# MP-Gadget/shenqi

Hardware: AMD Instinct MI355X
Metric: particle-steps/sec (grav+PM+SPH) at 256^3; rms force error vs ref (higher is better)
Workload: dtype f64

## Files before the change

include/shenqi_hip.h:

```cpp
#ifndef SHENQI_HIP_H
#define SHENQI_HIP_H

#include <stddef.h>
#include <stdint.h>

#ifdef __cplusplus
extern "C" {
#endif

#define SHQ_OK 0
#define SHQ_ERR_INVALID 1
#define SHQ_ERR_DEVICE 2
#define SHQ_ERR_NOMEM 3
#define SHQ_ERR_STATE 4
#define SHQ_ERR_NOCONV 5

#define SHQ_NGRAVTAB 512
#define SHQ_NMAXCHILD 8
#define SHQ_NODELISTLENGTH 4
#define SHQ_TIMEBINS 46

typedef struct shq_context shq_context;


// ... 363 lines not shown
    void *base;
    size_t elsize;
    int64_t numslots;
    size_t off_mintimebin, off_timebindynfric, off_jumptominpot;
    size_t off_dfaccel, off_df_surroundingvel, off_dragaccel;
    size_t off_minpotpos, off_minpotvel;
} shq_bh_dyn_view;
int shq_bh_dynamics_upload(shq_context *ctx, const shq_part_view *parts, const shq_bh_dyn_view *bh);
int shq_bh_dynamics_download(shq_context *ctx, const shq_part_view *parts, const shq_bh_dyn_view *bh);
int shq_set_bh_reposition(shq_context *ctx, int enabled);
int shq_kick_bh(shq_context *ctx, const double gravkick[SHQ_TIMEBINS + 1], const int32_t *active, int64_t nactive);
int shq_grav_short_run(shq_context *ctx, const shq_grav_params *params, const int32_t *active,
                       int64_t nactive, int update_potential, int walk_mode);
int shq_grav_short_run_range(shq_context *ctx, const shq_grav_params *params, int64_t first, int64_t count,
                             int update_potential, int walk_mode);
int shq_set_walk_stats(shq_context *ctx, int level);
int shq_set_walk_launch(shq_context *ctx, int persist, int leaf_ring);
int shq_set_walk_sparse(shq_context *ctx, int enable);
int shq_walk_pair_lean(shq_context *ctx);
int shq_set_walk_overlap(shq_context *ctx, int mode);
int shq_set_walk_addr(shq_context *ctx, int mode);
int shq_walk_last_addr(shq_context *ctx, int *mode);
int shq_walk_addr32_fits(int64_t numnodes);
int shq_walk_pair_status(shq_context *ctx, int64_t *recovered_launches, int64_t *stack_high_water, int64_t *last_mopped_tasks);
int shq_set_walk_debug(shq_context *ctx, int pair_spin_max, int pair_stack_cap);
int shq_set_tree_debug(shq_context *ctx, int64_t initial_node_cap);
int shq_tree_build_attempts(shq_context *ctx, int *attempts);
int shq_direct_force_sample(shq_context *ctx, const double *sample_pos, int64_t ns, int64_t nsrc, double BoxSize, double G, double h,
                            int repeat, double *accel);
int shq_grav_short_download(shq_context *ctx, double (*accel)[3], double *potential,
                            int64_t *ninteractions, shq_walk_stats *stats);
typedef struct shq_grav_query {
    double Pos[3];
    int32_t NodeList[4];
    double OldAcc;
} shq_grav_query;
typedef struct shq_grav_result {
    double Acc[3];
    double Potential;
} shq_grav_result;
int shq_grav_short_secondary(shq_context *ctx, const shq_grav_params *params, const shq_grav_query *queries, int64_t nq,
                             shq_grav_result *results, int64_t *ninteractions, int update_potential);
typedef struct shq_data_index {
    int32_t Task;
    int32_t Index;
    int32_t NodeList[4];
// ... 991 lines not shown
```

shenqi_amd/capi.py:

```python
import ctypes as C
import os

import numpy as np

_HERE = os.path.dirname(os.path.abspath(__file__))
LIBDIR = os.environ.get("SHQ_LIBDIR") or os.path.join(_HERE, "lib")
DATADIR = os.path.join(_HERE, "data")

NGRAVTAB = 512
NMAXCHILD = 8
NOFIELD = C.c_size_t(-1).value

WALK_EXACT = 0
WALK_GROUP = 1
WALK_AUTO = 2
WALK_TREE_ORDER = 0x100
WALK_DEFER_POSTPROCESS = 0x200


class ShqError(RuntimeError):
    """Non-zero status from the library (the shim's endrun() equivalent)."""


def _load(name):
# ... 394 lines not shown
GAS_NCOL = 28
hip.shq_gas_set_device.argtypes = [_vp, _vp, C.c_int64, C.c_int64]
hip.shq_gas_get_device.argtypes = [_vp, _vp, C.c_int64, C.c_int]
hip.shq_density_resident.argtypes = [_vp, C.POINTER(DensityParams), C.POINTER(SphStats)]
hip.shq_hydro_resident.argtypes = [_vp, C.POINTER(HydroParams), C.POINTER(SphStats)]
for _f in ("shq_gas_set_device", "shq_gas_get_device", "shq_density_resident", "shq_hydro_resident"):
    getattr(hip, _f).restype = C.c_int
hip.shq_set_walk_stats.argtypes = [_vp, C.c_int]
hip.shq_set_walk_stats.restype = C.c_int
hip.shq_set_walk_launch.argtypes = [_vp, C.c_int, C.c_int]
hip.shq_set_walk_launch.restype = C.c_int
hip.shq_set_walk_sparse.argtypes = [_vp, C.c_int]
hip.shq_set_walk_sparse.restype = C.c_int
hip.shq_walk_pair_lean.argtypes = [_vp]
hip.shq_walk_pair_lean.restype = C.c_int
hip.shq_set_walk_overlap.argtypes = [_vp, C.c_int]
hip.shq_set_walk_overlap.restype = C.c_int
hip.shq_set_walk_addr.argtypes = [_vp, C.c_int]
hip.shq_set_walk_addr.restype = C.c_int
hip.shq_walk_last_addr.argtypes = [_vp, C.POINTER(C.c_int)]
hip.shq_walk_last_addr.restype = C.c_int
hip.shq_walk_addr32_fits.argtypes = [C.c_int64]
hip.shq_walk_addr32_fits.restype = C.c_int
hip.shq_pm_set_fft_transposed.argtypes = [_vp, C.c_int]
hip.shq_pm_set_fft_transposed.restype = C.c_int
hip.shq_walk_pair_status.argtypes = [_vp, C.POINTER(C.c_int64), C.POINTER(C.c_int64), C.POINTER(C.c_int64)]
hip.shq_walk_pair_status.restype = C.c_int
hip.shq_set_walk_debug.argtypes = [_vp, C.c_int, C.c_int]
hip.shq_set_walk_debug.restype = C.c_int
hip.shq_set_tree_debug.argtypes = [_vp, C.c_int64]
hip.shq_set_tree_debug.restype = C.c_int
hip.shq_tree_build_attempts.argtypes = [_vp, C.POINTER(C.c_int)]
hip.shq_tree_build_attempts.restype = C.c_int
hip.shq_direct_force_sample.argtypes = [_vp, _vp, C.c_int64, C.c_int64, C.c_double, C.c_double, C.c_double, C.c_int, _vp]
hip.shq_direct_force_sample.restype = C.c_int
hip.shq_exchange_plan.argtypes = [_vp, C.POINTER(ExchangeLayout), _vp, C.c_int64, _vp, C.c_int, C.c_int, C.c_int64, C.POINTER(C.c_int64), C.POINTER(C.c_int64), _vp]
hip.shq_exchange_pack.argtypes = [_vp, C.POINTER(ExchangeLayout), _vp, _vp, C.c_int64, _vp, C.c_int, _vp, _vp]
hip.shq_exchange_unpack.argtypes = [_vp, C.POINTER(ExchangeLayout), _vp, C.c_int64, _vp, _vp, _vp, C.c_int]
hip.shq_slots_gc.argtypes = [_vp, C.POINTER(ExchangeLayout), _vp, C.POINTER(C.c_int64), C.c_int64, _vp, _vp, _vp]
hip.shq_slots_gc_sorted.argtypes = [_vp, C.POINTER(ExchangeLayout), _vp, C.POINTER(C.c_int64), C.c_int64, _vp, _vp, _vp]
hip.shq_slots_split_particles.argtypes = [_vp, C.POINTER(ExchangeLayout), C.POINTER(SpawnLayout), _vp, C.POINTER(C.c_int64), C.c_int64, _vp, _vp, C.c_int64, _vp]
hip.shq_slots_convert.argtypes = [_vp, C.POINTER(ExchangeLayout), _vp, C.c_int64, C.c_int64, _vp, _vp, _vp, _vp, C.c_int64, C.c_int]
hip.shq_make_particle_stars.argtypes = [_vp, C.POINTER(ExchangeLayout), C.POINTER(StarSpawnLayout), _vp, C.c_int64, C.c_int64, _vp, _vp, _vp, _vp, _vp, C.c_int64, C.c_double]
hip.shq_blackhole_make_seeds.argtypes = [_vp, C.POINTER(ExchangeLayout), C.POINTER(BhSeedLayout), _vp, C.c_int64, C.c_int64, _vp, _vp, _vp, _vp, _vp, C.c_int64,
                                         C.c_double, C.c_double]
hip.shq_bh_accretion.argtypes = [_vp, C.POINTER(TreeView), C.POINTER(PartView), C.POINTER(SphView), C.POINTER(BhSlotView), _vp, _vp, C.c_int64, C.POINTER(KickFactors),
# ... 926 lines not shown
```

shenqi_amd/csrc/capi.hip:

```cpp
#include "common.hpp"
#include <stdarg.h>
#include <string.h>
#include <stdlib.h>
#include <math.h>
#include <thread>
#include <atomic>
#include <algorithm>

static thread_local char g_err[1024] = "";

void shq_set_error(const char *fmt, ...)
{
    va_list ap;
    va_start(ap, fmt);
    vsnprintf(g_err, sizeof(g_err), fmt, ap);
    va_end(ap);
}

extern "C" const char *shq_last_error(void) { return g_err; }
extern "C" const char *shq_version(void) { return "shenqi_hip 0.1 (gfx950)"; }

namespace {

template <typename F> void parallel_for(int64_t n, F f)
// ... 286 lines not shown
    return SHQ_OK;
}

extern "C" int shq_set_walk_overlap(shq_context *ctx, int mode)
{
    SHQ_CHECK(ctx, SHQ_ERR_INVALID, "null context");
    SHQ_CHECK(mode >= 0 && mode <= 2, SHQ_ERR_INVALID, "walk overlap mode %d", mode);
    ctx->walk_overlap = mode;
    return SHQ_OK;
}

extern "C" int shq_set_walk_addr(shq_context *ctx, int mode)
{
    SHQ_CHECK(ctx, SHQ_ERR_INVALID, "null context");
    SHQ_CHECK(mode == 0 || mode == 1, SHQ_ERR_INVALID, "walk addr mode %d", mode);
    ctx->walk_addr = mode;
    return SHQ_OK;
}

extern "C" int shq_walk_last_addr(shq_context *ctx, int *mode)
{
    SHQ_CHECK(ctx && mode, SHQ_ERR_INVALID, "null argument");
    *mode = ctx->last_walk_addr32 ? 1 : 0;
    return SHQ_OK;
}

extern "C" int shq_walk_pair_lean(shq_context *ctx)
{
    SHQ_CHECK(ctx, SHQ_ERR_INVALID, "null context");
    if(!ctx->node_lean_checked || !ctx->node_lean_bad.ptr)
        return 0;
    SHQ_HIP(hipSetDevice(ctx->device));
    int bad = 1;
    SHQ_HIP(hipMemcpyAsync(&bad, ctx->node_lean_bad.ptr, sizeof(int), hipMemcpyDeviceToHost, ctx->stream));
    SHQ_HIP(hipStreamSynchronize(ctx->stream));
    return bad == 0 ? 1 : 0;
}

extern "C" int shq_set_walk_launch(shq_context *ctx, int persist, int leaf_ring)
{
    SHQ_CHECK(ctx && persist >= 0 && persist <= 2 && (leaf_ring == 0 || leaf_ring == 1), SHQ_ERR_INVALID, "walk launch: persist 0..2, leaf_ring 0 or 1");
    ctx->walk_persist = persist;
    ctx->walk_ring = leaf_ring;
    return SHQ_OK;
}

// ... 1182 lines not shown
```

shenqi_amd/csrc/common.hpp:

```cpp
#ifndef SHQ_COMMON_HPP
#define SHQ_COMMON_HPP

#include <hip/hip_runtime.h>
#include <hipfft/hipfft.h>
#include <stdint.h>
#include <stdio.h>
#include <string>
#include <vector>
#include "../../include/shenqi_hip.h"
#include "yields_math.hpp"
#include "cooling_math.hpp"

void shq_set_error(const char *fmt, ...);
void shq_heiii_run_free(shq_context *ctx);

#define SHQ_HIP(call)                                                                          \
    do {                                                                                       \
        hipError_t e_ = (call);                                                                \
        if(e_ != hipSuccess) {                                                                 \
            shq_set_error("%s:%d: %s failed: %s", __FILE__, __LINE__, #call, hipGetErrorString(e_)); \
            return (e_ == hipErrorOutOfMemory) ? SHQ_ERR_NOMEM : SHQ_ERR_DEVICE;               \
        }                                                                                      \
    } while(0)

// ... 406 lines not shown
    DevBuf<double> slab_fac;
    bool ps_slab = false;
    bool have_types = false;

    shq_walk_stats last_stats = {};
    int walk_variant = 3;
    int walk_stats = 0;
    int walk_persist = 1;
    int walk_ring = 1;
    int num_cus = 256;
    DevBuf<unsigned int> walk_tasks;
    DevBuf<int4> sp_items, sp_stack;
    DevBuf<int32_t> sp_count;
    DevBuf<int> sp_flags;
    PinBuf<int> sp_host;
    int sp_stack_cap = 0;
    unsigned sp_spin_max = 0;
    int walk_sparse = 1;
    DevBuf<int> node_lean_bad;
    bool node_lean_checked = false;
    int walk_overlap = 1;
    int walk_addr = 1;
    bool last_walk_addr32 = false;
    bool sp_check_pending = false;
    int xcd_k = 32;
    float last_walk_ms = 0;
    int last_walk_mode = 0;

    PinBuf<char> stage;

    bool uvbg_keep = false;
    int uvbg_n = 0;
    std::vector<float> uvbg_j21, uvbg_xhi;
    double uvbg_ms[4] = {0, 0, 0, 0};
    DevBuf<double> uvbg_tw, uvbg_tabs, uvbg_part;
    DevBuf<int> uvbg_flag;
    int uvbg_tw_n = 0, uvbg_tabs_n = 0, uvbg_tabs_nr = 0;
    shq_heiii_stats heiii_stats = {};
    struct HeiiiRun {
        int phase = 0;
        struct CallScope *sc = nullptr;
        int64_t n = 0;
        double box = 0, a3inv = 0, du = 0;
        int64_t m = 0, nrows = 0, n_flash = 0;
        int cur = 0;
        double4 *E[2] = {nullptr, nullptr}, *S = nullptr;
// ... 312 lines not shown
```

shenqi_amd/csrc/grav_walk.hip:

```cpp
#include "common.hpp"
#include "pm_readout.hpp"
#include <utility>
#include <stdlib.h>

namespace {

struct WalkArgs {
    const NodeG *nodeG;
    const double4 *posm;
    const double4 *posm_leaf;
    const double *oldacc;
    const int32_t *targets;
    const int32_t *qstart;
    double *acc;
    double *pot;
    int32_t *nint;
    GravStatsDev *stats;
    long long ntargets;
    int root;
    double Box, invBox, halfBox;
    double rcut, rcut2;
    double h, h2, h_inv, h3_inv;
    double inv_celldx;
    double errtol, bh2;
// ... 86 lines not shown
    }
    ax = fma(dx, fac, ax);
    ay = fma(dy, fac, ay);
    az = fma(dz, fac, az);
}

template <bool POT>
__device__ __forceinline__ void leaf_particle(const double4 *__restrict__ tab, const double4 q, double px, double py,
                                              double pz, const WalkArgs &a, double &ax, double &ay, double &az,
                                              double &pot, const unsigned long long wrapm)
{
    double ex = q.x - px, ey = q.y - py, ez = q.z - pz;
    if(wrapm != 0ull) {
        ex = wrapd(ex, a.Box, a.invBox);
        ey = wrapd(ey, a.Box, a.invBox);
        ez = wrapd(ez, a.Box, a.invBox);
    }
    const double rr2 = fma(ez, ez, fma(ey, ey, ex * ex));
    apply_accn<POT>(tab, ex, ey, ez, rr2, q.w, a, ax, ay, az, pot);
}

#if defined(__HIP_DEVICE_COMPILE__)
#define SHQ_CONSTANT_AS __attribute__((address_space(4)))
#else
#define SHQ_CONSTANT_AS
#endif
typedef const SHQ_CONSTANT_AS WalkArgs *WalkArgsK;
__device__ __forceinline__ WalkArgsK walk_cold_args()
{
    WalkArgsK kp = (WalkArgsK) __builtin_amdgcn_kernarg_segment_ptr();
    asm volatile("" : "+s"(kp));
    return kp;
}

template <typename T> __device__ __forceinline__ void agent_store(T *p, T v) { __hip_atomic_store(p, v, __ATOMIC_RELAXED, __HIP_MEMORY_SCOPE_AGENT); }
template <typename T> __device__ __forceinline__ T agent_load(const T *p) { return __hip_atomic_load(const_cast<T *>(p), __ATOMIC_RELAXED, __HIP_MEMORY_SCOPE_AGENT); }

__device__ __forceinline__ int walk_next_task(WalkArgsK c, int &region, int &tried)
{
    const int lg = c->task_run_log2;
    const int nwaves = (int) c->nwaves;
    unsigned int *counters = c->task_counters;
    while(tried < 8) {
        unsigned k = 0;
        if((threadIdx.x & 63) == 0)
            k = atomicAdd(&counters[16 * region], 1u);
        k = (unsigned) __builtin_amdgcn_readfirstlane((int) k);
        const unsigned t = ((((k >> lg) << 3) + (unsigned) region) << lg) | (k & ((1u << lg) - 1u));
        if(k < 0x40000000u && t < (unsigned) nwaves)
            return (int) t;
        region = (region + 1) & 7;
        tried++;
    }
    return -1;
}

#define SHQ_LEAF_RING 32
#ifndef SHQ_SPARSE_LANES
#define SHQ_SPARSE_LANES 8
#endif
#ifndef SHQ_SPARSE_CAP
#define SHQ_SPARSE_CAP 96
#endif
#define SHQ_SPARSE_STACK 4096
#define SHQ_SPARSE_SPIN (1u << 22)
#ifndef SHQ_PAIR_DEPTH2
#define SHQ_PAIR_DEPTH2 1
#endif
enum SpFlag {
    SP_OVERFLOW = 0,
    SP_GAVEUP = 1,
    SP_MOPPED = 2,
    SP_HIGHWATER = 3,
    SP_STICKY_ERROR = 8,
    SP_STICKY_RECOVERED = 9,
    SP_STICKY_HIGHWATER = 10,
    SP_TASK_COUNTER = 16
};
#define SP_TASK_DONE (-2)
#ifndef SHQ_PAIR_WAVES
#define SHQ_PAIR_WAVES 8
#define SHQ_PAIR_WG_PER_CU 2
// ... 384 lines not shown
            atomicAdd(&c.stats->lonely[3], (unsigned long long) l16m);
        }
    }
    }
    wave = PERSIST ? (long long) walk_next_task(walk_cold_args(), region, tried) : -1;
    }
}

struct LeanProducts { double rcuthl, mlen2, inside, wraplim; };
__device__ __forceinline__ LeanProducts lean_products(double mass, double len, double rcut, double Box)
{
    LeanProducts r;
    const double hl = 0.5 * len;
    r.rcuthl = rcut + hl;
    r.mlen2 = mass * len * len;
    r.inside = 0.6 * len;
    r.wraplim = fmax(0.5 * Box - hl, 0.0);
    return r;
}
__device__ __forceinline__ int lean_level(double rootlen, double len) { return (__double2hiint(rootlen) - __double2hiint(len)) >> 20; }

#pragma clang diagnostic push
#pragma clang diagnostic ignored "-Wpass-failed"
template <bool POT, int WAVES>
__device__ __forceinline__ void grav_pair_body(const WalkArgs &a)
{
    __shared__ double4 tab[SHQ_NGRAVTAB];
    __shared__ double4 tgt_all[WAVES][64];
    __shared__ double acc_all[WAVES][4][64];
    __shared__ int cnt_all[WAVES][64];
    __shared__ double bh_lvl[32];
    if(a.sp_mop && agent_load(a.sp_flags + SP_GAVEUP) == 0)
        return;
    const double rootlen = a.Box * 1.001;
    if(threadIdx.x < 32) {
        const double l = ldexp(rootlen, -(int) threadIdx.x);
        bh_lvl[threadIdx.x] = l * l / a.bh2;
    }
    const bool lean = __builtin_amdgcn_readfirstlane(a.sp_lean_bad ? (*a.sp_lean_bad == 0) : 0) != 0;
    for(int i = threadIdx.x; i < SHQ_NGRAVTAB; i += blockDim.x) {
        const int j = (i + 1 < SHQ_NGRAVTAB) ? i + 1 : i;
        const double f0 = a.tab_f[i], f1 = a.tab_f[j], p0 = a.tab_p[i], p1 = a.tab_p[j];
        tab[i] = i + 1 < SHQ_NGRAVTAB ? make_double4(f0, f1 - f0, p0, p1 - p0) : make_double4(0, 0, 0, 0);
    }
    __syncthreads();
    const int lane = threadIdx.x & 63, wv = threadIdx.x >> 6;
    double4 *const tgt = tgt_all[wv];
    double(*const acc)[64] = acc_all[wv];
    int *const cntl = cnt_all[wv];
    int4 *const stack = a.sp_stack + ((size_t) blockIdx.x * WAVES + wv) * (size_t) a.sp_stack_cap;
    int sp_high = 0;
    int mopped = 0;
    const unsigned long long below = (1ull << lane) - 1ull;
    long long w_sum = 0, w_min = 0x7fffffffffffll, w_max = 0;
    auto next_task = [&](long long prev) -> long long {
        if(a.sp_live) {
            unsigned k = 0;
            if(lane == 0)
                k = atomicAdd(a.sp_task, 1u);
            return (long long) (unsigned) __builtin_amdgcn_readfirstlane((int) k);
        }
        return prev < 0 ? (long long) blockIdx.x * WAVES + wv : prev + (long long) gridDim.x * WAVES;
    };
    for(long long task = next_task(-1); task < a.nwaves; task = next_task(task)) {
        const long long t = task * 64 + lane;
        const bool valid = t < a.ntargets;
        const long long pi = valid ? (a.targets ? (long long) a.targets[t] : t) : -1;
        const bool have = pi >= 0;
        int cnt = agent_load(&a.sp_count[task]);
        if(a.sp_mop) {
            if(__builtin_amdgcn_readfirstlane(cnt) == SP_TASK_DONE)
                continue;
            mopped++;
        }
        if(a.sp_live) {
            for(unsigned spin = 0; cnt < 0 && spin < a.sp_spin_max; spin++) {
                __builtin_amdgcn_s_sleep(32);
                cnt = agent_load(&a.sp_count[task]);
            }
            cnt = __builtin_amdgcn_readfirstlane(cnt);
            if(cnt < 0) {
                if(lane == 0)
                    agent_store(a.sp_flags + SP_GAVEUP, 1);
                break;
            }
        }
        int sp = 0;
        if(cnt > 0) {
            double4 me = make_double4(0, 0, 0, 0);
            if(have) {
                const double4 p = a.posm[pi];
                me = make_double4(p.x, p.y, p.z, a.errtol * agent_load(&a.oldacc[pi]));
            }
            tgt[lane] = me;
            for(int k = 0; k < 4; k++)
                acc[k][lane] = 0.0;
            cntl[lane] = 0;
            for(int k0 = 0; k0 < cnt; k0 += 64) {
                int4 mine = make_int4(0, 0, 0, 0);
                if(k0 + lane < cnt) {
                    const unsigned long long *const it = reinterpret_cast<const unsigned long long *>(a.sp_items + (task * SHQ_SPARSE_CAP + k0 + lane));
                    const unsigned long long lo = agent_load(it), hi = agent_load(it + 1);
                    mine = make_int4((int) (unsigned) lo, (int) (unsigned) (lo >> 32), (int) (unsigned) hi, (int) (unsigned) (hi >> 32));
                }
                const int kn = cnt - k0 < 64 ? cnt - k0 : 64;
                for(int k = 0; k < kn; k++) {
                    const int ix = __builtin_amdgcn_readlane(mine.x, k), iy = __builtin_amdgcn_readlane(mine.y, k);
                    const unsigned long long m = ((unsigned long long) (unsigned) __builtin_amdgcn_readlane(mine.w, k) << 32) |
                                                 (unsigned) __builtin_amdgcn_readlane(mine.z, k);
                    if((m >> lane) & 1ull)
                        stack[sp + __popcll(m & below)] = make_int4(ix, iy, lane, 0);
                    sp += __popcll(m);
                }
            }
            __builtin_amdgcn_fence(__ATOMIC_RELEASE, "wavefront");
            __builtin_amdgcn_wave_barrier();
        }
        struct PairLd {
            int node, end, slot, kind;
            double4 src;
            double cx, cy, cz, len;
            int nsib, nchild, ntype, ncount;
        };
        struct PairOut {
            int push_sib, push_child, child_end, leaf0, leafn;
        };
        auto pair_pop = [&](int base, int np, PairLd &p) {
            p.node = -1, p.end = -1, p.slot = 0, p.kind = 0;
            if(lane < np) {
                const int4 pr = stack[base + lane];
                p.node = pr.x, p.end = pr.y, p.slot = pr.z, p.kind = pr.w;
            }
        };
        auto pair_fetch = [&](PairLd &p) {
            p.src = make_double4(0, 0, 0, 0);
            p.cx = p.cy = p.cz = p.len = 0;
            p.nsib = -1, p.nchild = -1, p.ntype = 0, p.ncount = 0;
            if(p.node >= 0) {
                const double4 *const sp4 = p.kind == 1 ? a.posm_leaf + p.node : reinterpret_cast<const double4 *>(a.nodeG + p.node);
                p.src = *sp4;
                if(p.kind == 0) {
                    const NodeG *const nd = a.nodeG + p.node;
                    p.len = nd->len;
                    p.cx = nd->center[0], p.cy = nd->center[1], p.cz = nd->center[2];
                    p.nsib = nd->sibling, p.nchild = nd->child, p.ntype = nd->type, p.ncount = nd->count;
                }
            }
        };
        auto pair_eval = [&](const PairLd &p, PairOut &o) {
            o.push_sib = -1, o.push_child = -1, o.child_end = -1, o.leaf0 = 0, o.leafn = 0;
            double ax = 0, ay = 0, az = 0, pot = 0;
            const bool live = p.node >= 0, isnode = live && p.kind == 0;
            double wraplim = 0, rcut2 = 0, rcuthl = 0, mlen2 = 0, bhlim = 0, inside = 0;
            if(isnode) {
                if(lean) {
                    const LeanProducts lp = lean_products(p.src.w, p.len, a.rcut, a.Box);
                    rcuthl = lp.rcuthl, mlen2 = lp.mlen2, inside = lp.inside, wraplim = lp.wraplim, rcut2 = a.rcut2;
                    bhlim = bh_lvl[lean_level(rootlen, p.len) & 31];
                } else {
                    const NodeG *const nd = a.nodeG + p.node;
                    bhlim = nd->bhlim, mlen2 = nd->mlen2, inside = nd->inside, rcut2 = nd->rcut2, wraplim = nd->wraplim, rcuthl = nd->rcuthl;
                }
            }
            const double4 tg = tgt[p.slot];
            double dx = p.src.x - tg.x, dy = p.src.y - tg.y, dz = p.src.z - tg.z;
            double ux = p.cx - tg.x, uy = p.cy - tg.y, uz = p.cz - tg.z;
            double cmax = fmax(fmax(fabs(ux), fabs(uy)), fabs(uz));
            const bool nwrap = isnode && __double2hiint(wraplim) >= 0 && cmax >= wraplim;
            if(nwrap || (live && !isnode)) {
                dx = wrapd(dx, a.Box, a.invBox);
                dy = wrapd(dy, a.Box, a.invBox);
                dz = wrapd(dz, a.Box, a.invBox);
            }
            if(nwrap) {
                ux = wrapd(ux, a.Box, a.invBox);
                uy = wrapd(uy, a.Box, a.invBox);
                uz = wrapd(uz, a.Box, a.invBox);
                cmax = fmax(fmax(fabs(ux), fabs(uy)), fabs(uz));
            }
            const double r2 = dx * dx + dy * dy + dz * dz;
            bool ev = live && !isnode;
            if(isnode) {
                const bool keep = !(r2 > rcut2 && cmax > rcuthl);
                const bool open = (!a.useBH && mlen2 > r2 * r2 * tg.w) || r2 < bhlim || cmax < inside;
                ev = keep && !open;
                if(keep && open) {
                    if(p.ntype == SHQ_NODE_NODE_TYPE) {
                        o.push_child = p.nchild;
                        o.child_end = p.nsib;
                    } else if(p.ntype == SHQ_PARTICLE_NODE_TYPE) {
                        o.leaf0 = p.nchild;
                        o.leafn = p.ncount;
                    }
                }
                if(p.nsib != p.end && p.nsib >= 0)
                    o.push_sib = p.nsib;
            }
            if(ev) {
                apply_accn<POT, true>(tab, dx, dy, dz, r2, p.src.w, a, ax, ay, az, pot);
                atomicAdd(&acc[0][p.slot], ax);
                atomicAdd(&acc[1][p.slot], ay);
                atomicAdd(&acc[2][p.slot], az);
                if(POT)
                    atomicAdd(&acc[3][p.slot], pot);
                atomicAdd(&cntl[p.slot], 1);
            }
        };
        auto push_nodes = [&](int what, int what_end, int slot) {
            const unsigned long long m = shq_ballot(what >= 0);
            if(what >= 0)
                stack[sp + __popcll(m & below)] = make_int4(what, what_end, slot, 0);
            sp += __popcll(m);
        };
        auto push_leaves = [&](int leaf0, int leafn, int slot) {
            if(shq_ballot(leafn > 0) != 0ull) {
                const unsigned long long b0 = shq_ballot((leafn & 1) != 0), b1 = shq_ballot((leafn & 2) != 0),
                                         b2 = shq_ballot((leafn & 4) != 0), b3 = shq_ballot((leafn & 8) != 0);
                const int off = __popcll(b0 & below) + 2 * __popcll(b1 & below) + 4 * __popcll(b2 & below) + 8 * __popcll(b3 & below);
                for(int k = 0; k < SHQ_NMAXCHILD; k++) {
                    if(shq_ballot(k < leafn) == 0ull)
                        break;
                    if(k < leafn)
                        stack[sp + off + k] = make_int4(leaf0 + k, -1, slot, 1);
                }
                sp += __popcll(b0) + 2 * __popcll(b1) + 4 * __popcll(b2) + 8 * __popcll(b3);
            }
        };
        while(sp > 0) {
            const int npa = sp < 64 ? sp : 64;
            sp -= npa;
            const int npb = SHQ_PAIR_DEPTH2 ? (sp < 64 ? sp : 64) : 0;
            sp -= npb;
            PairLd pa, pb;
            PairOut oa, ob;
            pair_pop(sp + npb, npa, pa);
            if(npb > 0)
                pair_pop(sp, npb, pb);
            pair_fetch(pa);
            if(npb > 0)
                pair_fetch(pb);
            pair_eval(pa, oa);
            if(npb > 0)
                pair_eval(pb, ob);
            push_nodes(oa.push_sib, pa.end, pa.slot);
            if(npb > 0)
                push_nodes(ob.push_sib, pb.end, pb.slot);
            push_nodes(oa.push_child, oa.child_end, pa.slot);
            if(npb > 0)
                push_nodes(ob.push_child, ob.child_end, pb.slot);
            push_leaves(oa.leaf0, oa.leafn, pa.slot);
            if(npb > 0)
                push_leaves(ob.leaf0, ob.leafn, pb.slot);
            sp_high = sp > sp_high ? sp : sp_high;
            if(sp > a.sp_stack_cap - 1280) {
                if(lane == 0) {
                    agent_store(a.sp_flags + SP_OVERFLOW, 1);
                    atomicOr(a.sp_flags + SP_STICKY_ERROR, 1);
                }
                sp = 0;
            }
            __builtin_amdgcn_fence(__ATOMIC_RELEASE, "wavefront");
            __builtin_amdgcn_wave_barrier();
        }
        long long nint = 0;
        if(have) {
            nint = agent_load(&a.nint[pi]);
            if(cnt > 0) {
                __builtin_amdgcn_fence(__ATOMIC_ACQUIRE, "wavefront");
                a.acc[3 * pi + 0] = agent_load(&a.acc[3 * pi + 0]) + acc[0][lane];
                a.acc[3 * pi + 1] = agent_load(&a.acc[3 * pi + 1]) + acc[1][lane];
                a.acc[3 * pi + 2] = agent_load(&a.acc[3 * pi + 2]) + acc[2][lane];
                if(POT)
                    a.pot[pi] = agent_load(&a.pot[pi]) + acc[3][lane];
                nint += (long long) cntl[lane];
                a.nint[pi] = (int32_t) nint;
            }
        }
        long long mn = have ? nint : 0x7fffffffffffll, mx = have ? nint : 0, sm = have ? nint : 0;
        for(int off = 32; off > 0; off >>= 1) {
            const long long o1 = __shfl_xor(mn, off), o2 = __shfl_xor(mx, off), o3 = __shfl_xor(sm, off);
            mn = o1 < mn ? o1 : mn;
            mx = o2 > mx ? o2 : mx;
            sm += o3;
        }
        w_sum += sm;
        w_min = mn < w_min ? mn : w_min;
        w_max = mx > w_max ? mx : w_max;
        if(lane == 0)
            agent_store(&a.sp_count[task], (int32_t) SP_TASK_DONE);
        __builtin_amdgcn_wave_barrier();
    }
    if(lane == 0 && a.stats) {
        atomicAdd(&a.stats->ninteractions, (unsigned long long) w_sum);
        atomicMin(&a.stats->min_int, w_min);
        atomicMax(&a.stats->max_int, w_max);
    }
    if(lane == 0 && sp_high > 0) {
        atomicMax(a.sp_flags + SP_HIGHWATER, sp_high);
        atomicMax(a.sp_flags + SP_STICKY_HIGHWATER, sp_high);
    }
    if(lane == 0 && mopped > 0)
        atomicAdd(a.sp_flags + SP_MOPPED, mopped);
    if(a.sp_mop && blockIdx.x == 0 && threadIdx.x == 0)
        atomicAdd(a.sp_flags + SP_STICKY_RECOVERED, 1);
}

template <bool POT> __global__ __launch_bounds__(256) __attribute__((amdgpu_waves_per_eu(4, 4))) void grav_pair_kernel_live(const WalkArgs a) { grav_pair_body<POT, 4>(a); }
template <bool POT> __global__ __launch_bounds__(64 * SHQ_PAIR_WAVES) __attribute__((amdgpu_waves_per_eu(SHQ_PAIR_EU, SHQ_PAIR_EU))) void grav_pair_kernel(const WalkArgs a)
{
    grav_pair_body<POT, SHQ_PAIR_WAVES>(a);
}

#pragma clang diagnostic pop

__global__ void grav_postprocess_kernel(const int32_t *targets, long long ntargets, const double4 *posm, double *acc,
                                        double *pot, double *treeacc, double G, double h, double cbrtrho0,
                                        int update_potential)
{
    const long long t = (long long) blockIdx.x * blockDim.x + threadIdx.x;
    if(t >= ntargets)
        return;
    const long long i = targets ? (long long) targets[t] : t;
    if(i < 0)
        return;
    const double a0 = acc[3 * i + 0] * G, a1 = acc[3 * i + 1] * G, a2 = acc[3 * i + 2] * G;
    acc[3 * i + 0] = a0;
    acc[3 * i + 1] = a1;
    acc[3 * i + 2] = a2;
    if(update_potential) {
        treeacc[3 * i + 0] = a0;
        treeacc[3 * i + 1] = a1;
        treeacc[3 * i + 2] = a2;
        const double m = posm[i].w;
// ... 78 lines not shown
        grav_walk_exact_kernel<POT, PREFETCH, LEAFB, (POT && !PREFETCH && LEAFB == 2) ? 2 : 1, BH><<<grid, block, 0, stream>>>(a);
    else if(stats)
        grav_walk_exact_kernel<POT, PREFETCH, LEAFB, 1, BH><<<grid, block, 0, stream>>>(a);
    else if(persist && !PREFETCH && LEAFB == 2 && block.x == 512)
        grav_walk_exact_kernel<POT, PREFETCH, LEAFB, 0, BH, false, (!PREFETCH && LEAFB == 2), (!PREFETCH && LEAFB == 2)><<<grid, block, dyn_lds, stream>>>(a);
    else if(persist && !PREFETCH && LEAFB == 2)
        grav_walk_exact_kernel<POT, PREFETCH, LEAFB, 0, BH, false, (!PREFETCH && LEAFB == 2)><<<grid, block, dyn_lds, stream>>>(a);
    else
        grav_walk_exact_kernel<POT, PREFETCH, LEAFB, 0, BH><<<grid, block, 0, stream>>>(a);
    return false;
}

template <bool POT, bool PREFETCH, int LEAFB>
bool launch_variant(int stats, bool persist, dim3 grid, dim3 block, hipStream_t stream, const WalkArgs &a, size_t dyn_lds = 0, bool addr32 = false)
{
    if(a.useBH)
        return launch_variant_bh<POT, PREFETCH, LEAFB, true>(stats, persist, grid, block, stream, a, dyn_lds, addr32);
    return launch_variant_bh<POT, PREFETCH, LEAFB, false>(stats, persist, grid, block, stream, a, dyn_lds, addr32);
}

}

extern "C" int shq_walk_addr32_fits(int64_t numnodes) { return (numnodes >= 0 && numnodes + 1 <= ((int64_t) 1 << 25)) ? 1 : 0; }

void shq_launch_stats_init(shq_context *ctx) { stats_init_kernel<<<1, 1, 0, ctx->stream>>>(ctx->gstats.ptr); }

void shq_fill_node_walk_params(shq_context *ctx, const shq_grav_params *p)
{
    if((ctx->node_rcut != p->Rcut || ctx->node_bh2 != p->BHOpeningAngle2) && ctx->numnodes > 0) {
        const long long n = ctx->numnodes + 1;
        int *lean_bad = nullptr;
        if(ctx->node_lean_bad.reserve(16) == SHQ_OK && hipMemsetAsync(ctx->node_lean_bad.ptr, 0, sizeof(int) * 16, ctx->stream) == hipSuccess)
            lean_bad = ctx->node_lean_bad.ptr;
        ctx->node_lean_checked = lean_bad != nullptr;
        fill_rcuthl_kernel<<<dim3((unsigned) ((n + 255) / 256)), dim3(256), 0, ctx->stream>>>(ctx->nodeG.ptr, n, p->Rcut, p->BHOpeningAngle2, p->BoxSize, lean_bad);
        ctx->node_rcut = p->Rcut;
        ctx->node_bh2 = p->BHOpeningAngle2;
    }
}

static void fill_walk_args(shq_context *ctx, const shq_grav_params *p, WalkArgs &a)
{
    shq_fill_node_walk_params(ctx, p);
    a.nodeG = ctx->nodeG.ptr;
    a.posm = ctx->posm.ptr;
    a.posm_leaf = ctx->posm_leaf.ptr;
// ... 312 lines not shown
    bool used32 = false;
    if(update_potential) {
        switch(variant) {
        case 0: launch_variant<true, false, 4>(stats, persist, grid, block, ctx->stream, a); break;
        case 1: launch_variant<true, false, 2>(stats, persist, grid, block, ctx->stream, a); break;
        case 2: launch_variant<true, false, 4>(stats, persist, grid, block, ctx->stream, a); break;
        default: used32 = launch_variant<true, false, 2>(stats, persist, grid, block, ctx->stream, a, dyn_lds, addr32); break;
        }
    } else {
        switch(variant) {
        case 0: launch_variant<false, false, 4>(stats, persist, grid, block, ctx->stream, a); break;
        case 1: launch_variant<false, false, 2>(stats, persist, grid, block, ctx->stream, a); break;
        case 2: launch_variant<false, false, 4>(stats, persist, grid, block, ctx->stream, a); break;
        default: used32 = launch_variant<false, false, 2>(stats, persist, grid, block, ctx->stream, a, dyn_lds, addr32); break;
        }
    }
    SHQ_HIP(hipGetLastError());
    ctx->last_walk_addr32 = used32;
    if(sparse) {
        hipStream_t ps = live ? ctx->stream_pair : ctx->stream;
        if(live)
            SHQ_HIP(hipStreamWaitEvent(ps, ctx->ev_pair_fork, 0));
        const dim3 pg((unsigned) pair_blocks);
        if(live) {
            if(update_potential)
                grav_pair_kernel_live<true><<<pg, dim3(256), 0, ps>>>(a);
            else
                grav_pair_kernel_live<false><<<pg, dim3(256), 0, ps>>>(a);
        } else if(update_potential)
            grav_pair_kernel<true><<<pg, dim3(64 * SHQ_PAIR_WAVES), 0, ps>>>(a);
        else
            grav_pair_kernel<false><<<pg, dim3(64 * SHQ_PAIR_WAVES), 0, ps>>>(a);
        SHQ_HIP(hipGetLastError());
        if(live) {
            SHQ_HIP(hipEventRecord(ctx->ev_pair_join, ps));
            SHQ_HIP(hipStreamWaitEvent(ctx->stream, ctx->ev_pair_join, 0));
            WalkArgs m = a;
            m.sp_live = 0;
            m.sp_mop = 1;
            const dim3 mg((unsigned) mop_blocks);
            if(update_potential)
                grav_pair_kernel<true><<<mg, dim3(64 * SHQ_PAIR_WAVES), 0, ctx->stream>>>(m);
            else
                grav_pair_kernel<false><<<mg, dim3(64 * SHQ_PAIR_WAVES), 0, ctx->stream>>>(m);
            SHQ_HIP(hipGetLastError());
        }
        SHQ_HIP(hipMemcpyAsync(ctx->sp_host.ptr, ctx->sp_flags.ptr + SP_STICKY_ERROR, sizeof(int) * 8, hipMemcpyDeviceToHost, ctx->stream));
        ctx->sp_check_pending = true;
    }
    SHQ_HIP(hipEventRecord(ctx->ev_end[SHQ_T_WALK], ctx->stream));
    if(swap_meshes) {
        std::swap(ctx->mesh.ptr, ctx->mesh_alt.ptr);
        std::swap(ctx->mesh.cap, ctx->mesh_alt.cap);
    }
    if(scrubbed)
        ctx->mesh_zeroed = true;
    return SHQ_OK;
}

int shq_launch_grav_postprocess(shq_context *ctx, const shq_grav_params *p, const int32_t *d_active, int64_t ntargets,
                                int update_potential, int64_t first)
{
    if(ntargets == 0)
        return SHQ_OK;
    const int threads = 256;
    const long long blocks = (ntargets + threads - 1) / threads;
    grav_postprocess_kernel<<<dim3((unsigned) blocks), dim3(threads), 0, ctx->stream>>>(
// ... 98 lines not shown
```

Baseline: 433.0 million.

## Use 32-bit offsets and wave-mask logic in sparse pair gravity walk

Adds an A32 variant of the pair-walk kernel that addresses the node table, leaf positions and per-wave stack with 32-bit byte offsets from uniform bases. Push and evaluation decisions become wave-wide ballot masks, with inverse_ballot masking and mbcnt-based prefix counts, and the leaf push is unrolled into mask-guarded stores. Per-task min/max/sum reductions move out of the task loop, and SHQ_SPARSE_LANES rises from 8 to 12. The aim is lower VGPR/SGPR pressure and less 64-bit address arithmetic and divergence, at the cost of more code and a size-fit check that falls back to 64-bit addressing.

```diff
diff --git a/include/shenqi_hip.h b/include/shenqi_hip.h
--- a/include/shenqi_hip.h
+++ b/include/shenqi_hip.h
@@ -409,6 +409,8 @@
 int shq_set_walk_addr(shq_context *ctx, int mode);
 int shq_walk_last_addr(shq_context *ctx, int *mode);
 int shq_walk_addr32_fits(int64_t numnodes);
+int shq_pair_addr32_fits(int64_t numnodes, int64_t leaf_slots, int64_t stack_cap);
+int shq_walk_last_pair_addr(shq_context *ctx, int *mode);
 int shq_walk_pair_status(shq_context *ctx, int64_t *recovered_launches, int64_t *stack_high_water, int64_t *last_mopped_tasks);
 int shq_set_walk_debug(shq_context *ctx, int pair_spin_max, int pair_stack_cap);
 int shq_set_tree_debug(shq_context *ctx, int64_t initial_node_cap);
diff --git a/shenqi_amd/capi.py b/shenqi_amd/capi.py
--- a/shenqi_amd/capi.py
+++ b/shenqi_amd/capi.py
@@ -440,6 +440,10 @@
 hip.shq_walk_last_addr.restype = C.c_int
 hip.shq_walk_addr32_fits.argtypes = [C.c_int64]
 hip.shq_walk_addr32_fits.restype = C.c_int
+hip.shq_pair_addr32_fits.argtypes = [C.c_int64, C.c_int64, C.c_int64]
+hip.shq_pair_addr32_fits.restype = C.c_int
+hip.shq_walk_last_pair_addr.argtypes = [_vp, C.POINTER(C.c_int)]
+hip.shq_walk_last_pair_addr.restype = C.c_int
 hip.shq_pm_set_fft_transposed.argtypes = [_vp, C.c_int]
 hip.shq_pm_set_fft_transposed.restype = C.c_int
 hip.shq_walk_pair_status.argtypes = [_vp, C.POINTER(C.c_int64), C.POINTER(C.c_int64), C.POINTER(C.c_int64)]
diff --git a/shenqi_amd/csrc/capi.hip b/shenqi_amd/csrc/capi.hip
--- a/shenqi_amd/csrc/capi.hip
+++ b/shenqi_amd/csrc/capi.hip
@@ -332,6 +332,13 @@
 {
     SHQ_CHECK(ctx && mode, SHQ_ERR_INVALID, "null argument");
     *mode = ctx->last_walk_addr32 ? 1 : 0;
+    return SHQ_OK;
+}
+
+extern "C" int shq_walk_last_pair_addr(shq_context *ctx, int *mode)
+{
+    SHQ_CHECK(ctx && mode, SHQ_ERR_INVALID, "null argument");
+    *mode = ctx->last_pair_addr32 ? 1 : 0;
     return SHQ_OK;
 }
 
diff --git a/shenqi_amd/csrc/common.hpp b/shenqi_amd/csrc/common.hpp
--- a/shenqi_amd/csrc/common.hpp
+++ b/shenqi_amd/csrc/common.hpp
@@ -452,6 +452,7 @@
     int walk_overlap = 1;
     int walk_addr = 1;
     bool last_walk_addr32 = false;
+    bool last_pair_addr32 = false;
     bool sp_check_pending = false;
     int xcd_k = 32;
     float last_walk_ms = 0;
diff --git a/shenqi_amd/csrc/grav_walk.hip b/shenqi_amd/csrc/grav_walk.hip
--- a/shenqi_amd/csrc/grav_walk.hip
+++ b/shenqi_amd/csrc/grav_walk.hip
@@ -132,8 +132,10 @@
 
 #if defined(__HIP_DEVICE_COMPILE__)
 #define SHQ_CONSTANT_AS __attribute__((address_space(4)))
+#define SHQ_GLOBAL_AS __attribute__((address_space(1)))
 #else
 #define SHQ_CONSTANT_AS
+#define SHQ_GLOBAL_AS
 #endif
 typedef const SHQ_CONSTANT_AS WalkArgs *WalkArgsK;
 __device__ __forceinline__ WalkArgsK walk_cold_args()
@@ -167,7 +169,7 @@
 
 #define SHQ_LEAF_RING 32
 #ifndef SHQ_SPARSE_LANES
-#define SHQ_SPARSE_LANES 8
+#define SHQ_SPARSE_LANES 12
 #endif
 #ifndef SHQ_SPARSE_CAP
 #define SHQ_SPARSE_CAP 96
@@ -598,7 +600,7 @@
 
 #pragma clang diagnostic push
 #pragma clang diagnostic ignored "-Wpass-failed"
-template <bool POT, int WAVES>
+template <bool POT, int WAVES, bool A32>
 __device__ __forceinline__ void grav_pair_body(const WalkArgs &a)
 {
     __shared__ double4 tab[SHQ_NGRAVTAB];
@@ -624,10 +626,30 @@
     double4 *const tgt = tgt_all[wv];
     double(*const acc)[64] = acc_all[wv];
     int *const cntl = cnt_all[wv];
-    int4 *const stack = a.sp_stack + ((size_t) blockIdx.x * WAVES + wv) * (size_t) a.sp_stack_cap;
+    const int wslot = __builtin_amdgcn_readfirstlane((int) (blockIdx.x * WAVES + wv));
+    int4 *const stack = a.sp_stack + (size_t) wslot * (size_t) a.sp_stack_cap;
+    auto stk = [&](int i) -> int4 & {
+        if constexpr(A32)
+            return *reinterpret_cast<int4 *>(reinterpret_cast<char *>(stack) + ((unsigned) i << 4));
+        else
+            return stack[i];
+    };
+    unsigned nb_lo = 0, nb_hi = 0, lb_lo = 0, lb_hi = 0;
+    if constexpr(A32) {
+        asm volatile("v_mov_b32 %0, %1" : "=v"(nb_lo) : "s"((unsigned) (size_t) a.nodeG));
+        asm volatile("v_mov_b32 %0, %1" : "=v"(nb_hi) : "s"((unsigned) ((size_t) a.nodeG >> 32)));
+        asm volatile("v_mov_b32 %0, %1" : "=v"(lb_lo) : "s"((unsigned) (size_t) a.posm_leaf));
+        asm volatile("v_mov_b32 %0, %1" : "=v"(lb_hi) : "s"((unsigned) ((size_t) a.posm_leaf >> 32)));
+    }
+    auto rec = [&](int i) -> const NodeG * {
+        if constexpr(A32)
+            return reinterpret_cast<const NodeG *>(reinterpret_cast<const char *>(a.nodeG) + ((unsigned) i << 7));
+        else
+            return a.nodeG + i;
+    };
     int sp_high = 0;
     int mopped = 0;
-    const unsigned long long below = (1ull << lane) - 1ull;
+    auto below = [](unsigned long long m) { return (int) __builtin_amdgcn_mbcnt_hi((unsigned) (m >> 32), __builtin_amdgcn_mbcnt_lo((unsigned) m, 0u)); };
     long long w_sum = 0, w_min = 0x7fffffffffffll, w_max = 0;
     auto next_task = [&](long long prev) -> long long {
         if(a.sp_live) {
@@ -636,25 +658,24 @@
                 k = atomicAdd(a.sp_task, 1u);
             return (long long) (unsigned) __builtin_amdgcn_readfirstlane((int) k);
         }
-        return prev < 0 ? (long long) blockIdx.x * WAVES + wv : prev + (long long) gridDim.x * WAVES;
+        return prev < 0 ? (long long) wslot : prev + (long long) gridDim.x * WAVES;
     };
     for(long long task = next_task(-1); task < a.nwaves; task = next_task(task)) {
         const long long t = task * 64 + lane;
         const bool valid = t < a.ntargets;
         const long long pi = valid ? (a.targets ? (long long) a.targets[t] : t) : -1;
         const bool have = pi >= 0;
-        int cnt = agent_load(&a.sp_count[task]);
+        int cnt = __builtin_amdgcn_readfirstlane(agent_load(&a.sp_count[task]));
         if(a.sp_mop) {
-            if(__builtin_amdgcn_readfirstlane(cnt) == SP_TASK_DONE)
+            if(cnt == SP_TASK_DONE)
                 continue;
             mopped++;
         }
         if(a.sp_live) {
             for(unsigned spin = 0; cnt < 0 && spin < a.sp_spin_max; spin++) {
                 __builtin_amdgcn_s_sleep(32);
-                cnt = agent_load(&a.sp_count[task]);
-            }
-            cnt = __builtin_amdgcn_readfirstlane(cnt);
+                cnt = __builtin_amdgcn_readfirstlane(agent_load(&a.sp_count[task]));
+            }
             if(cnt < 0) {
                 if(lane == 0)
                     agent_store(a.sp_flags + SP_GAVEUP, 1);
@@ -685,7 +706,7 @@
                     const unsigned long long m = ((unsigned long long) (unsigned) __builtin_amdgcn_readlane(mine.w, k) << 32) |
                                                  (unsigned) __builtin_amdgcn_readlane(mine.z, k);
                     if((m >> lane) & 1ull)
-                        stack[sp + __popcll(m & below)] = make_int4(ix, iy, lane, 0);
+                        stk(sp + below(m)) = make_int4(ix, iy, lane, 0);
                     sp += __popcll(m);
                 }
             }
@@ -694,121 +715,162 @@
         }
         struct PairLd {
             int node, end, slot, kind;
+            unsigned long long livem, nodem;
+            int nidx;
             double4 src;
             double cx, cy, cz, len;
             int nsib, nchild, ntype, ncount;
         };
         struct PairOut {
-            int push_sib, push_child, child_end, leaf0, leafn;
+            unsigned long long sibm, childm, leafm;
         };
         auto pair_pop = [&](int base, int np, PairLd &p) {
-            p.node = -1, p.end = -1, p.slot = 0, p.kind = 0;
-            if(lane < np) {
-                const int4 pr = stack[base + lane];
-                p.node = pr.x, p.end = pr.y, p.slot = pr.z, p.kind = pr.w;
-            }
+            const int4 pr = stk(base + (lane < np ? lane : np - 1));
+            p.node = pr.x, p.end = pr.y, p.slot = pr.z, p.kind = pr.w;
+            p.livem = shq_ballot(lane < np);
         };
         auto pair_fetch = [&](PairLd &p) {
-            p.src = make_double4(0, 0, 0, 0);
-            p.cx = p.cy = p.cz = p.len = 0;
-            p.nsib = -1, p.nchild = -1, p.ntype = 0, p.ncount = 0;
-            if(p.node >= 0) {
-                const double4 *const sp4 = p.kind == 1 ? a.posm_leaf + p.node : reinterpret_cast<const double4 *>(a.nodeG + p.node);
+            const bool isn = p.kind == 0;
+            p.nodem = shq_ballot(isn) & p.livem;
+            p.nidx = isn ? p.node : 0;
+            if constexpr(A32) {
+                const unsigned long long b = ((unsigned long long) (isn ? nb_hi : lb_hi) << 32) | (isn ? nb_lo : lb_lo);
+                p.src = *reinterpret_cast<const SHQ_GLOBAL_AS double4 *>(b + ((unsigned) p.node << (isn ? 7 : 5)));
+            } else {
+                const double4 *const sp4 = isn ? reinterpret_cast<const double4 *>(a.nodeG + p.node) : a.posm_leaf + p.node;
                 p.src = *sp4;
-                if(p.kind == 0) {
-                    const NodeG *const nd = a.nodeG + p.node;
-                    p.len = nd->len;
-                    p.cx = nd->center[0], p.cy = nd->center[1], p.cz = nd->center[2];
-                    p.nsib = nd->sibling, p.nchild = nd->child, p.ntype = nd->type, p.ncount = nd->count;
-                }
+            }
+            if(p.nodem != 0ull) {
+                const NodeG *const nd = rec(p.nidx);
+                p.len = nd->len;
+                p.cx = nd->center[0], p.cy = nd->center[1], p.cz = nd->center[2];
+                p.nsib = nd->sibling, p.nchild = nd->child, p.ntype = nd->type, p.ncount = nd->count;
             }
         };
         auto pair_eval = [&](const PairLd &p, PairOut &o) {
-            o.push_sib = -1, o.push_child = -1, o.child_end = -1, o.leaf0 = 0, o.leafn = 0;
-            double ax = 0, ay = 0, az = 0, pot = 0;
-            const bool live = p.node >= 0, isnode = live && p.kind == 0;
-            double wraplim = 0, rcut2 = 0, rcuthl = 0, mlen2 = 0, bhlim = 0, inside = 0;
-            if(isnode) {
+            o.sibm = o.childm = o.leafm = 0ull;
+            const unsigned long long partm = p.livem & ~p.nodem;
+            const double4 tg = tgt[p.slot];
+            double dx = p.src.x - tg.x, dy = p.src.y - tg.y, dz = p.src.z - tg.z;
+            double ux, uy, uz, cmax, wraplim, rcut2, rcuthl, mlen2, bhlim, inside;
+            unsigned long long nwrapm = 0ull;
+            if(p.nodem != 0ull) {
                 if(lean) {
                     const LeanProducts lp = lean_products(p.src.w, p.len, a.rcut, a.Box);
                     rcuthl = lp.rcuthl, mlen2 = lp.mlen2, inside = lp.inside, wraplim = lp.wraplim, rcut2 = a.rcut2;
                     bhlim = bh_lvl[lean_level(rootlen, p.len) & 31];
+                    asm volatile("" : "+v"(bhlim));
                 } else {
-                    const NodeG *const nd = a.nodeG + p.node;
+                    const NodeG *const nd = rec(p.nidx);
                     bhlim = nd->bhlim, mlen2 = nd->mlen2, inside = nd->inside, rcut2 = nd->rcut2, wraplim = nd->wraplim, rcuthl = nd->rcuthl;
                 }
-            }
-            const double4 tg = tgt[p.slot];
-            double dx = p.src.x - tg.x, dy = p.src.y - tg.y, dz = p.src.z - tg.z;
-            double ux = p.cx - tg.x, uy = p.cy - tg.y, uz = p.cz - tg.z;
-            double cmax = fmax(fmax(fabs(ux), fabs(uy)), fabs(uz));
-            const bool nwrap = isnode && __double2hiint(wraplim) >= 0 && cmax >= wraplim;
-            if(nwrap || (live && !isnode)) {
-                dx = wrapd(dx, a.Box, a.invBox);
-                dy = wrapd(dy, a.Box, a.invBox);
-                dz = wrapd(dz, a.Box, a.invBox);
-            }
-            if(nwrap) {
-                ux = wrapd(ux, a.Box, a.invBox);
-                uy = wrapd(uy, a.Box, a.invBox);
-                uz = wrapd(uz, a.Box, a.invBox);
+                ux = p.cx - tg.x, uy = p.cy - tg.y, uz = p.cz - tg.z;
                 cmax = fmax(fmax(fabs(ux), fabs(uy)), fabs(uz));
-            }
-            const double r2 = dx * dx + dy * dy + dz * dz;
-            bool ev = live && !isnode;
-            if(isnode) {
-                const bool keep = !(r2 > rcut2 && cmax > rcuthl);
-                const bool open = (!a.useBH && mlen2 > r2 * r2 * tg.w) || r2 < bhlim || cmax < inside;
-                ev = keep && !open;
-                if(keep && open) {
-                    if(p.ntype == SHQ_NODE_NODE_TYPE) {
-                        o.push_child = p.nchild;
-                        o.child_end = p.nsib;
-                    } else if(p.ntype == SHQ_PARTICLE_NODE_TYPE) {
-                        o.leaf0 = p.nchild;
-                        o.leafn = p.ncount;
+                nwrapm = shq_ballot(__double2hiint(wraplim) >= 0) & shq_ballot(cmax >= wraplim) & p.nodem;
+            }
+            const unsigned long long dwrapm = nwrapm | partm;
+            if(dwrapm != 0ull) {
+                if(__builtin_amdgcn_inverse_ballot_w64(dwrapm)) {
+                    dx = wrapd(dx, a.Box, a.invBox);
+                    dy = wrapd(dy, a.Box, a.invBox);
+                    dz = wrapd(dz, a.Box, a.invBox);
+                }
+            }
+            const double r2 = fma(dz, dz, fma(dx, dx, dy * dy));
+            unsigned long long evm = partm;
+            if(p.nodem != 0ull) {
+                if(nwrapm != 0ull) {
+                    if(__builtin_amdgcn_inverse_ballot_w64(nwrapm)) {
+                        ux = wrapd(ux, a.Box, a.invBox);
+                        uy = wrapd(uy, a.Box, a.invBox);
+                        uz = wrapd(uz, a.Box, a.invBox);
+                        cmax = fmax(fmax(fabs(ux), fabs(uy)), fabs(uz));
                     }
                 }
-                if(p.nsib != p.end && p.nsib >= 0)
-                    o.push_sib = p.nsib;
-            }
-            if(ev) {
-                apply_accn<POT, true>(tab, dx, dy, dz, r2, p.src.w, a, ax, ay, az, pot);
-                atomicAdd(&acc[0][p.slot], ax);
-                atomicAdd(&acc[1][p.slot], ay);
-                atomicAdd(&acc[2][p.slot], az);
-                if(POT)
-                    atomicAdd(&acc[3][p.slot], pot);
-                atomicAdd(&cntl[p.slot], 1);
+                const unsigned long long keepm = p.nodem & ~(shq_ballot(r2 > rcut2) & shq_ballot(cmax > rcuthl));
+                unsigned long long openm = shq_ballot(r2 < bhlim) | shq_ballot(cmax < inside);
+                if(!a.useBH)
+                    openm |= shq_ballot(mlen2 > r2 * r2 * tg.w);
+                const unsigned long long kopenm = keepm & openm;
+                evm |= keepm & ~openm;
+                if(kopenm != 0ull) {
+                    o.childm = kopenm & shq_ballot(p.ntype == SHQ_NODE_NODE_TYPE);
+                    o.leafm = kopenm & shq_ballot(p.ntype == SHQ_PARTICLE_NODE_TYPE);
+                }
+                o.sibm = p.nodem & shq_ballot(p.nsib != p.end) & shq_ballot(p.nsib >= 0);
+            }
+            if(evm != 0ull) {
+                if(__builtin_amdgcn_inverse_ballot_w64(evm)) {
+                    double ax = 0, ay = 0, az = 0, pot = 0;
+                    apply_accn<POT, true>(tab, dx, dy, dz, r2, p.src.w, a, ax, ay, az, pot);
+                    atomicAdd(&acc[0][p.slot], ax);
+                    atomicAdd(&acc[1][p.slot], ay);
+                    atomicAdd(&acc[2][p.slot], az);
+                    if(POT)
+                        atomicAdd(&acc[3][p.slot], pot);
+                    atomicAdd(&cntl[p.slot], 1);
+                }
             }
         };
-        auto push_nodes = [&](int what, int what_end, int slot) {
-            const unsigned long long m = shq_ballot(what >= 0);
-            if(what >= 0)
-                stack[sp + __popcll(m & below)] = make_int4(what, what_end, slot, 0);
-            sp += __popcll(m);
+        auto push_nodes = [&](unsigned long long m, int what, int what_end, int slot) {
+            if(m != 0ull) {
+                if(__builtin_amdgcn_inverse_ballot_w64(m))
+                    stk(sp + below(m)) = make_int4(what, what_end, slot, 0);
+                sp += __popcll(m);
+            }
         };
-        auto push_leaves = [&](int leaf0, int leafn, int slot) {
-            if(shq_ballot(leafn > 0) != 0ull) {
-                const unsigned long long b0 = shq_ballot((leafn & 1) != 0), b1 = shq_ballot((leafn & 2) != 0),
-                                         b2 = shq_ballot((leafn & 4) != 0), b3 = shq_ballot((leafn & 8) != 0);
-                const int off = __popcll(b0 & below) + 2 * __popcll(b1 & below) + 4 * __popcll(b2 & below) + 8 * __popcll(b3 & below);
-                for(int k = 0; k < SHQ_NMAXCHILD; k++) {
-                    if(shq_ballot(k < leafn) == 0ull)
-                        break;
-                    if(k < leafn)
-                        stack[sp + off + k] = make_int4(leaf0 + k, -1, slot, 1);
+        auto push_leaves = [&](unsigned long long m, int leaf0, int leafn, int slot) {
+            if(m != 0ull) {
+                const unsigned long long b0 = m & shq_ballot((leafn & 1) != 0), b1 = m & shq_ballot((leafn & 2) != 0),
+                                         b2 = m & shq_ballot((leafn & 4) != 0), b3 = m & shq_ballot((leafn & 8) != 0);
+                const int at = sp + below(b0) + 2 * below(b1) + 4 * below(b2) + 8 * below(b3);
+                const unsigned atb = (unsigned) at << 4;
+                auto put = [&](unsigned long long g, int k) {
+                    if(__builtin_amdgcn_inverse_ballot_w64(g)) {
+                        if constexpr(A32)
+                            *reinterpret_cast<int4 *>(reinterpret_cast<char *>(stack) + ((size_t) atb + 16u * (unsigned) k)) = make_int4(leaf0 + k, -1, slot, 1);
+                        else
+                            stk(at + k) = make_int4(leaf0 + k, -1, slot, 1);
+                    }
+                };
+                const unsigned long long g1 = b3 | b2 | b1, g0 = g1 | b0, g2 = b3 | b2 | (b1 & b0), g3 = b3 | b2, g4 = b3 | (b2 & (b1 | b0)), g5 = b3 | (b2 & b1),
+                                         g6 = b3 | (b2 & b1 & b0), g7 = b3;
+                if(g0 != 0ull) {
+                    put(g0, 0);
+                    if(g1 != 0ull) {
+                        put(g1, 1);
+                        if(g2 != 0ull) {
+                            put(g2, 2);
+                            if(g3 != 0ull) {
+                                put(g3, 3);
+                                if(g4 != 0ull) {
+                                    put(g4, 4);
+                                    if(g5 != 0ull) {
+                                        put(g5, 5);
+                                        if(g6 != 0ull) {
+                                            put(g6, 6);
+                                            if(g7 != 0ull)
+                                                put(g7, 7);
+                                        }
+                                    }
+                                }
+                            }
+                        }
+                    }
                 }
                 sp += __popcll(b0) + 2 * __popcll(b1) + 4 * __popcll(b2) + 8 * __popcll(b3);
             }
         };
         while(sp > 0) {
+            sp = __builtin_amdgcn_readfirstlane(sp);
             const int npa = sp < 64 ? sp : 64;
             sp -= npa;
             const int npb = SHQ_PAIR_DEPTH2 ? (sp < 64 ? sp : 64) : 0;
             sp -= npb;
             PairLd pa, pb;
             PairOut oa, ob;
+            pb.livem = pb.nodem = 0ull;
+            ob.sibm = ob.childm = ob.leafm = 0ull;
             pair_pop(sp + npb, npa, pa);
             if(npb > 0)
                 pair_pop(sp, npb, pb);
@@ -818,15 +880,15 @@
             pair_eval(pa, oa);
             if(npb > 0)
                 pair_eval(pb, ob);
-            push_nodes(oa.push_sib, pa.end, pa.slot);
+            push_nodes(oa.sibm, pa.nsib, pa.end, pa.slot);
             if(npb > 0)
-                push_nodes(ob.push_sib, pb.end, pb.slot);
-            push_nodes(oa.push_child, oa.child_end, pa.slot);
+                push_nodes(ob.sibm, pb.nsib, pb.end, pb.slot);
+            push_nodes(oa.childm, pa.nchild, pa.nsib, pa.slot);
             if(npb > 0)
-                push_nodes(ob.push_child, ob.child_end, pb.slot);
-            push_leaves(oa.leaf0, oa.leafn, pa.slot);
+                push_nodes(ob.childm, pb.nchild, pb.nsib, pb.slot);
+            push_leaves(oa.leafm, pa.nchild, pa.ncount, pa.slot);
             if(npb > 0)
-                push_leaves(ob.leaf0, ob.leafn, pb.slot);
+                push_leaves(ob.leafm, pb.nchild, pb.ncount, pb.slot);
             sp_high = sp > sp_high ? sp : sp_high;
             if(sp > a.sp_stack_cap - 1280) {
                 if(lane == 0) {
@@ -851,20 +913,19 @@
                 nint += (long long) cntl[lane];
                 a.nint[pi] = (int32_t) nint;
             }
-        }
-        long long mn = have ? nint : 0x7fffffffffffll, mx = have ? nint : 0, sm = have ? nint : 0;
-        for(int off = 32; off > 0; off >>= 1) {
-            const long long o1 = __shfl_xor(mn, off), o2 = __shfl_xor(mx, off), o3 = __shfl_xor(sm, off);
-            mn = o1 < mn ? o1 : mn;
-            mx = o2 > mx ? o2 : mx;
-            sm += o3;
-        }
-        w_sum += sm;
-        w_min = mn < w_min ? mn : w_min;
-        w_max = mx > w_max ? mx : w_max;
+            w_sum += nint;
+            w_min = nint < w_min ? nint : w_min;
+            w_max = nint > w_max ? nint : w_max;
+        }
         if(lane == 0)
             agent_store(&a.sp_count[task], (int32_t) SP_TASK_DONE);
         __builtin_amdgcn_wave_barrier();
+    }
+    for(int off = 32; off > 0; off >>= 1) {
+        const long long o1 = __shfl_xor(w_min, off), o2 = __shfl_xor(w_max, off), o3 = __shfl_xor(w_sum, off);
+        w_min = o1 < w_min ? o1 : w_min;
+        w_max = o2 > w_max ? o2 : w_max;
+        w_sum += o3;
     }
     if(lane == 0 && a.stats) {
         atomicAdd(&a.stats->ninteractions, (unsigned long long) w_sum);
@@ -881,10 +942,30 @@
         atomicAdd(a.sp_flags + SP_STICKY_RECOVERED, 1);
 }
 
-template <bool POT> __global__ __launch_bounds__(256) __attribute__((amdgpu_waves_per_eu(4, 4))) void grav_pair_kernel_live(const WalkArgs a) { grav_pair_body<POT, 4>(a); }
-template <bool POT> __global__ __launch_bounds__(64 * SHQ_PAIR_WAVES) __attribute__((amdgpu_waves_per_eu(SHQ_PAIR_EU, SHQ_PAIR_EU))) void grav_pair_kernel(const WalkArgs a)
-{
-    grav_pair_body<POT, SHQ_PAIR_WAVES>(a);
+template <bool POT, bool A32> __global__ __launch_bounds__(256) __attribute__((amdgpu_waves_per_eu(4, 4))) void grav_pair_kernel_live(const WalkArgs a)
+{
+    grav_pair_body<POT, 4, A32>(a);
+}
+template <bool POT, bool A32>
+__global__ __launch_bounds__(64 * SHQ_PAIR_WAVES) __attribute__((amdgpu_waves_per_eu(SHQ_PAIR_EU, SHQ_PAIR_EU))) void grav_pair_kernel(const WalkArgs a)
+{
+    grav_pair_body<POT, SHQ_PAIR_WAVES, A32>(a);
+}
+void launch_pair(bool live_form, bool pot, bool a32, dim3 grid, hipStream_t st, const WalkArgs &a)
+{
+    if(live_form) {
+        const dim3 b(256);
+        if(pot)
+            a32 ? grav_pair_kernel_live<true, true><<<grid, b, 0, st>>>(a) : grav_pair_kernel_live<true, false><<<grid, b, 0, st>>>(a);
+        else
+            a32 ? grav_pair_kernel_live<false, true><<<grid, b, 0, st>>>(a) : grav_pair_kernel_live<false, false><<<grid, b, 0, st>>>(a);
+    } else {
+        const dim3 b(64 * SHQ_PAIR_WAVES);
+        if(pot)
+            a32 ? grav_pair_kernel<true, true><<<grid, b, 0, st>>>(a) : grav_pair_kernel<true, false><<<grid, b, 0, st>>>(a);
+        else
+            a32 ? grav_pair_kernel<false, true><<<grid, b, 0, st>>>(a) : grav_pair_kernel<false, false><<<grid, b, 0, st>>>(a);
+    }
 }
 
 #pragma clang diagnostic pop
@@ -1009,6 +1090,11 @@
 }
 
 extern "C" int shq_walk_addr32_fits(int64_t numnodes) { return (numnodes >= 0 && numnodes + 1 <= ((int64_t) 1 << 25)) ? 1 : 0; }
+extern "C" int shq_pair_addr32_fits(int64_t numnodes, int64_t leaf_slots, int64_t stack_cap)
+{
+    const int64_t reach = (int64_t) 1 << 32;
+    return (shq_walk_addr32_fits(numnodes) != 0 && leaf_slots >= 0 && leaf_slots <= (reach >> 5) && stack_cap >= 0 && stack_cap <= (reach >> 4)) ? 1 : 0;
+}
 
 void shq_launch_stats_init(shq_context *ctx) { stats_init_kernel<<<1, 1, 0, ctx->stream>>>(ctx->gstats.ptr); }
 
@@ -1367,15 +1453,9 @@
         if(live)
             SHQ_HIP(hipStreamWaitEvent(ps, ctx->ev_pair_fork, 0));
         const dim3 pg((unsigned) pair_blocks);
-        if(live) {
-            if(update_potential)
-                grav_pair_kernel_live<true><<<pg, dim3(256), 0, ps>>>(a);
-            else
-                grav_pair_kernel_live<false><<<pg, dim3(256), 0, ps>>>(a);
-        } else if(update_potential)
-            grav_pair_kernel<true><<<pg, dim3(64 * SHQ_PAIR_WAVES), 0, ps>>>(a);
-        else
-            grav_pair_kernel<false><<<pg, dim3(64 * SHQ_PAIR_WAVES), 0, ps>>>(a);
+        const bool pair32 = ctx->walk_addr != 0 && shq_pair_addr32_fits(ctx->numnodes, ctx->ntreeparts + SHQ_NMAXCHILD, a.sp_stack_cap) != 0;
+        ctx->last_pair_addr32 = pair32;
+        launch_pair(live, update_potential != 0, pair32, pg, ps, a);
         SHQ_HIP(hipGetLastError());
         if(live) {
             SHQ_HIP(hipEventRecord(ctx->ev_pair_join, ps));
@@ -1384,10 +1464,7 @@
             m.sp_live = 0;
             m.sp_mop = 1;
             const dim3 mg((unsigned) mop_blocks);
-            if(update_potential)
-                grav_pair_kernel<true><<<mg, dim3(64 * SHQ_PAIR_WAVES), 0, ctx->stream>>>(m);
-            else
-                grav_pair_kernel<false><<<mg, dim3(64 * SHQ_PAIR_WAVES), 0, ctx->stream>>>(m);
+            launch_pair(false, update_potential != 0, pair32, mg, ctx->stream, m);
             SHQ_HIP(hipGetLastError());
         }
         SHQ_HIP(hipMemcpyAsync(ctx->sp_host.ptr, ctx->sp_flags.ptr + SP_STICKY_ERROR, sizeof(int) * 8, hipMemcpyDeviceToHost, ctx->stream));
```

Result: faster. 446.7 million, median of 6 (+3.2%).
